# CompVis/unsupervised-part-segmentation

Measured on AMD Instinct MI355X. Metric: images/sec training (CUB 128x128, 10 parts), higher is better.
Workload: dtype bf16

## Files before the change

unsupervised-part-segmentation_amd/csrc/conv_igemm.hip:

```cpp
#include <stdlib.h>

#include "common.h"

namespace {

constexpr int BM = 128;
constexpr int RS = 80;

template <typename T> struct Mma;

template <> struct Mma<bf16> {
    template <int TM, int TN>
    __device__ static inline void chunk(const unsigned char* a_base, const unsigned char* b_base, int lane,
                                        f32x16 (&acc)[TM][TN]) {
        const int r = lane & 31, h = lane >> 5;
#pragma unroll
        for (int ks = 0; ks < 2; ++ks) {
            bf16x8 a[TM], b[TN];
#pragma unroll
            for (int i = 0; i < TM; ++i) a[i] = *(const bf16x8*)(a_base + (i * 32 + r) * RS + ks * 32 + h * 16);
#pragma unroll
            for (int j = 0; j < TN; ++j) b[j] = *(const bf16x8*)(b_base + (j * 32 + r) * RS + ks * 32 + h * 16);
#pragma unroll
            for (int i = 0; i < TM; ++i)
#pragma unroll
                for (int j = 0; j < TN; ++j)
                    acc[i][j] = __builtin_amdgcn_mfma_f32_32x32x16_bf16(a[i], b[j], acc[i][j], 0, 0, 0);
        }
    }
};

template <> struct Mma<f16> {
    template <int TM, int TN>
    __device__ static inline void chunk(const unsigned char* a_base, const unsigned char* b_base, int lane,
                                        f32x16 (&acc)[TM][TN]) {
        const int r = lane & 31, h = lane >> 5;
#pragma unroll
        for (int ks = 0; ks < 2; ++ks) {
            f16x8 a[TM], b[TN];
#pragma unroll
            for (int i = 0; i < TM; ++i) a[i] = *(const f16x8*)(a_base + (i * 32 + r) * RS + ks * 32 + h * 16);
#pragma unroll
            for (int j = 0; j < TN; ++j) b[j] = *(const f16x8*)(b_base + (j * 32 + r) * RS + ks * 32 + h * 16);
#pragma unroll
            for (int i = 0; i < TM; ++i)
#pragma unroll
                for (int j = 0; j < TN; ++j)
                    acc[i][j] = __builtin_amdgcn_mfma_f32_32x32x16_f16(a[i], b[j], acc[i][j], 0, 0, 0);
        }
    }
};

template <> struct Mma<float> {
    template <int TM, int TN>
    __device__ static inline void chunk(const unsigned char* a_base, const unsigned char* b_base, int lane,
                                        f32x16 (&acc)[TM][TN]) {
        const int r = lane & 31, h = lane >> 5;
        f32x4 a[TM][2], b[TN][2];
#pragma unroll
        for (int i = 0; i < TM; ++i) {
            a[i][0] = *(const f32x4*)(a_base + (i * 32 + r) * RS + h * 32);
            a[i][1] = *(const f32x4*)(a_base + (i * 32 + r) * RS + h * 32 + 16);
        }
#pragma unroll
        for (int j = 0; j < TN; ++j) {
            b[j][0] = *(const f32x4*)(b_base + (j * 32 + r) * RS + h * 32);
            b[j][1] = *(const f32x4*)(b_base + (j * 32 + r) * RS + h * 32 + 16);
        }
#pragma unroll
        for (int kk = 0; kk < 8; ++kk)
#pragma unroll
            for (int i = 0; i < TM; ++i)
#pragma unroll
                for (int j = 0; j < TN; ++j)
                    acc[i][j] = __builtin_amdgcn_mfma_f32_32x32x2f32(a[i][kk >> 2][kk & 3], b[j][kk >> 2][kk & 3],
                                                                     acc[i][j], 0, 0, 0);
    }
};

__device__ inline int tap_dy_of(unsigned long long off, int t) { return (int)((off >> (4 * t + 2)) & 3) - 1; }
__device__ inline int tap_dx_of(unsigned long long off, int t) { return (int)((off >> (4 * t)) & 3) - 1; }
__device__ inline int tap_w_of(unsigned long long wi, int t) { return (int)((wi >> (4 * t)) & 15); }

struct ConvK {
    int n, hi, wi, ci, ldi, ho, wo, co, co_fill, ldo, out_h, out_w, out_sy, out_sx, out_oy, out_ox, in_sy, in_sx;
    int ntaps, kh, kw, act_in, out_f32, dact_kind, ldr, ldd, out_act, res_act;
    float act_slope;
    unsigned long long tap_off, tap_wi;
    const void* in; const void* w; void* out;
    const float* bias; const float* coord_tab; const void* res; const void* dact;
    float* ws; int splits, stages_per_split, ldw;
};

template <typename T, int BN, int CPS>
__global__ __launch_bounds__(256, (CPS == 1 ? 3 : 2)) void conv_igemm_kernel(const ConvK p, const int M, const int ntn,
                                                         const int kchunks) {
    constexpr int EPC = Chunk<T>::N;
    constexpr int BK = 4 * EPC;
    constexpr int WN = (BN == 32) ? 1 : 2;
    constexpr int WM = 4 / WN;
    constexpr int TM = BM / WM / 32;
    constexpr int TN = BN / WN / 32;
    constexpr int BROWS = (BN + 63) / 64;

    constexpr int SUB = (BM + BN) * RS;
    constexpr int STAGE = CPS * SUB;
    extern __shared__ __attribute__((aligned(16))) unsigned char smem[];
    long long* rowpix = (long long*)(smem + 2 * STAGE);
    int* rowaux = (int*)(rowpix + BM);

    const int tid = threadIdx.x, lane = tid & 63, wid = tid >> 6;
    const float act_ns = ups_slope_eff(p.act_in, p.act_slope);
    const float dact_ns = ups_slope_eff(p.dact_kind, p.act_slope);
    const int nt = blockIdx.x % ntn, mt = blockIdx.x / ntn;
    const int wm = wid / WN, wn = wid % WN;

    const T* __restrict__ in = (const T*)p.in;
    const T* __restrict__ w = (const T*)p.w;
    const int hw_o = p.ho * p.wo;

    const int chunk = tid & 3, r0 = tid >> 2;
    int iy0[2], ix0[2];
    long long ibase[2];
    bool rv[2];
#pragma unroll
    for (int q = 0; q < 2; ++q) {
        const int m = mt * BM + r0 + 64 * q;
        rv[q] = m < M;
        const int mm = rv[q] ? m : 0;
        const int img = mm / hw_o, rem = mm - img * hw_o;
        const int i = rem / p.wo, j = rem - i * p.wo;
        iy0[q] = i * p.in_sy;
        ix0[q] = j * p.in_sx;
        ibase[q] = (long long)img * p.hi * p.wi;
    }
    const bool b_thread = (BN >= 64) || (tid < 128);

    struct RSet { uint4 a0[CPS], a1[CPS], b0[CPS], b1[CPS]; } s0, s1;
    const uint4 zero4 = make_uint4(0u, 0u, 0u, 0u);
    const int iy00 = iy0[0], iy01 = iy0[1], ix00 = ix0[0], ix01 = ix0[1];
    const long long ib0 = ibase[0], ib1 = ibase[1];
    const bool rv0 = rv[0], rv1 = rv[1];
    const int total = p.ntaps * kchunks;

    auto load_a = [&](bool rvq, int iy, int ix, long long ib, int dy, int dx, int koff, bool kok) __attribute__((always_inline)) -> uint4 {
        const int y = iy + dy, x = ix + dx;
        const bool ok = rvq && kok && (unsigned)y < (unsigned)p.hi && (unsigned)x < (unsigned)p.wi;
        uint4 v = zero4;
        if (ok) v = *(const uint4*)(in + ((ib + (long long)y * p.wi + x) * p.ldi + koff));
        return v;
    };
    auto load_b = [&](const T* wt, int c, bool live) __attribute__((always_inline)) -> uint4 {
        uint4 v = zero4;
        if (live && b_thread && c < p.co) v = *(const uint4*)(wt + (long long)c * BK + chunk * EPC);
        return v;
    };
    auto load_stage = [&](RSet& q, int sidx) __attribute__((always_inline)) {
#pragma unroll
        for (int u = 0; u < CPS; ++u) {
            const int c = sidx * CPS + u;
            const bool live = c < total;
            const int cs = live ? c : 0;
            const int t = cs / kchunks, kc = cs - t * kchunks;
            const int koff = kc * BK + chunk * EPC;
            const bool kok = live && koff < p.ci;
            const int dy = tap_dy_of(p.tap_off, t), dx = tap_dx_of(p.tap_off, t);
            q.a0[u] = load_a(rv0, iy00, ix00, ib0, dy, dx, koff, kok);
            q.a1[u] = load_a(rv1, iy01, ix01, ib1, dy, dx, koff, kok);
            const T* wt = w + ((long long)tap_w_of(p.tap_wi, t) * kchunks + kc) * p.co * BK;
            q.b0[u] = load_b(wt, nt * BN + r0, live);
            if (BROWS > 1) q.b1[u] = load_b(wt, nt * BN + r0 + 64, live);
        }
    };
    auto act_u4 = [&](uint4 u) __attribute__((always_inline)) -> uint4 {
        if (p.act_in != UPS_ACT_NONE) {
            u = ups_act_chunk(u, act_ns, (T*)nullptr);
        }
        return u;
    };
    auto store_stage = [&](const RSet& q, unsigned char* st) __attribute__((always_inline)) {
#pragma unroll
        for (int u = 0; u < CPS; ++u) {
            unsigned char* As = st + u * SUB;
            unsigned char* Bs = As + BM * RS;
            *(uint4*)(As + r0 * RS + chunk * 16) = act_u4(q.a0[u]);
            *(uint4*)(As + (r0 + 64) * RS + chunk * 16) = act_u4(q.a1[u]);
            if (b_thread) {
                *(uint4*)(Bs + r0 * RS + chunk * 16) = q.b0[u];
                if (BROWS > 1) *(uint4*)(Bs + (r0 + 64) * RS + chunk * 16) = q.b1[u];
            }
        }
    };

    f32x16 acc[TM][TN];
#pragma unroll
    for (int i = 0; i < TM; ++i)
#pragma unroll
        for (int j = 0; j < TN; ++j)
#pragma unroll
            for (int e = 0; e < 16; ++e) acc[i][j][e] = 0.f;

    const int all_stages = (total + CPS - 1) / CPS;
    const int sbase = p.splits > 1 ? blockIdx.y * p.stages_per_split : 0;
    const int nstages = p.splits > 1 ? min(p.stages_per_split, all_stages - sbase) : all_stages;
    load_stage(s0, sbase);
    store_stage(s0, smem);
    if (nstages > 1) load_stage(s1, sbase + 1);
    __syncthreads();
    auto iter = [&](int sidx, RSet& ld_set, const RSet& st_set) __attribute__((always_inline)) {
        if (sidx + 2 < nstages) load_stage(ld_set, sbase + sidx + 2);
        const unsigned char* st = smem + (sidx & 1) * STAGE;
#pragma unroll
        for (int u = 0; u < CPS; ++u)
            Mma<T>::template chunk<TM, TN>(st + u * SUB + (wm * TM * 32) * RS, st + u * SUB + BM * RS + (wn * TN * 32) * RS,
                                           lane, acc);
        if (sidx + 1 < nstages) store_stage(st_set, smem + ((sidx + 1) & 1) * STAGE);
        __syncthreads();
    };
    for (int sidx = 0; sidx < nstages; sidx += 2) {
        iter(sidx, s0, s1);
        if (sidx + 1 < nstages) iter(sidx + 1, s1, s0);
    }

    if (p.splits > 1) {
        float* wsp = p.ws + ((long long)blockIdx.y * M) * p.ldw;
#pragma unroll
        for (int tn = 0; tn < TN; ++tn) {
            const int col = nt * BN + (wn * TN + tn) * 32 + (lane & 31);
#pragma unroll
            for (int tm = 0; tm < TM; ++tm)
#pragma unroll
                for (int e = 0; e < 16; ++e) {
                    const int m = mt * BM + (wm * TM + tm) * 32 + (e & 3) + 8 * (e >> 2) + 4 * (lane >> 5);
                    if (m < M) wsp[(long long)m * p.ldw + col] = acc[tm][tn][e];
                }
        }
        return;
    }
    if (tid < BM) {
        const int m = mt * BM + tid;
        long long pix = -1;
        int cls = 0, i = 0, j = 0;
        if (m < M) {
            const int img = m / hw_o, rem = m - img * hw_o;
            i = rem / p.wo; j = rem - i * p.wo;
            pix = ((long long)img * p.out_h + (i * p.out_sy + p.out_oy)) * p.out_w + (j * p.out_sx + p.out_ox);
            if (p.coord_tab) {
                int ym = 0, xm = 0;
                for (int r = 0; r < p.kh; ++r) ym |= ((unsigned)(i * p.in_sy + tap_dy_of(p.tap_off, r * p.kw)) < (unsigned)p.hi) << r;
                for (int s = 0; s < p.kw; ++s) xm |= ((unsigned)(j * p.in_sx + tap_dx_of(p.tap_off, s)) < (unsigned)p.wi) << s;
                cls = ym * 8 + xm;
            }
        }
        rowpix[tid] = pix;
        rowaux[tid * 3 + 0] = cls; rowaux[tid * 3 + 1] = j; rowaux[tid * 3 + 2] = i;
    }
    __syncthreads();

    T* __restrict__ outT = (T*)p.out;
    float* __restrict__ outF = (float*)p.out;
    const T* __restrict__ res = (const T*)p.res;
    const T* __restrict__ dact = (const T*)p.dact;
#pragma unroll
    for (int tn = 0; tn < TN; ++tn) {
        const int col = nt * BN + (wn * TN + tn) * 32 + (lane & 31);
        const bool cvalid = col < p.co;
        const bool cfill = col < p.co_fill;
        const float bias = (cvalid && p.bias) ? p.bias[col] : 0.f;
#pragma unroll
        for (int tm = 0; tm < TM; ++tm) {
#pragma unroll
            for (int e = 0; e < 16; ++e) {
                const int rl = (wm * TM + tm) * 32 + (e & 3) + 8 * (e >> 2) + 4 * (lane >> 5);
                const long long pix = rowpix[rl];
                if (pix < 0 || !cfill) continue;
                float v = 0.f;
                if (cvalid) {
                    v = acc[tm][tn][e] + bias;
                    if (p.coord_tab) {
                        const float* tb = p.coord_tab + (long long)rowaux[rl * 3] * 3 * p.co + col;
                        v += tb[0] + (float)rowaux[rl * 3 + 1] * tb[p.co] + (float)rowaux[rl * 3 + 2] * tb[2 * p.co];
                    }
                    if (dact) v *= (ld_as_float<T>(dact + pix * p.ldd + col) > 0.f) ? 1.f : dact_ns;
                    if (res) {
                        float rr = ld_as_float<T>(res + pix * p.ldr + col);
                        if (p.res_act) rr = rr > 0.f ? rr : rr / p.act_slope;
                        v += rr;
                    }
                    if (p.out_act) v = ups_vmax(v, ups_slope_eff(p.out_act, p.act_slope) * v);
                }
                if (p.out_f32) outF[pix * p.ldo + col] = v;
                else st_from_float<T>(outT + pix * p.ldo + col, v);
            }
        }
    }
}

template <typename T>
__global__ __launch_bounds__(256) void igemm_splitk_epilogue(const ConvK p, const int M) {
    const long long gid = (long long)blockIdx.x * blockDim.x + threadIdx.x;
    const int col = (int)(gid % p.co_fill);
    const long long m = gid / p.co_fill;
    if (m >= M) return;
    float v = 0.f;
    for (int sp = 0; sp < p.splits; ++sp) v += p.ws[((long long)sp * M + m) * p.ldw + col];
    const int hw_o = p.ho * p.wo;
    const int img = (int)(m / hw_o), rem = (int)(m - (long long)img * hw_o);
    const int i = rem / p.wo, j = rem - i * p.wo;
    const long long pix = ((long long)img * p.out_h + (i * p.out_sy + p.out_oy)) * p.out_w + (j * p.out_sx + p.out_ox);
    const bool cvalid = col < p.co;
    if (cvalid) {
        if (p.bias) v += p.bias[col];
        if (p.coord_tab) {
            int ym = 0, xm = 0;
            for (int r = 0; r < p.kh; ++r) ym |= ((unsigned)(i * p.in_sy + tap_dy_of(p.tap_off, r * p.kw)) < (unsigned)p.hi) << r;
            for (int q = 0; q < p.kw; ++q) xm |= ((unsigned)(j * p.in_sx + tap_dx_of(p.tap_off, q)) < (unsigned)p.wi) << q;
            const float* tb = p.coord_tab + (long long)(ym * 8 + xm) * 3 * p.co + col;
            v += tb[0] + (float)j * tb[p.co] + (float)i * tb[2 * p.co];
        }
        if (p.dact) v *= (ld_as_float<T>((const T*)p.dact + pix * p.ldd + col) > 0.f) ? 1.f : ups_slope_eff(p.dact_kind, p.act_slope);
        if (p.res) {
            float rr = ld_as_float<T>((const T*)p.res + pix * p.ldr + col);
            if (p.res_act) rr = rr > 0.f ? rr : rr / p.act_slope;
            v += rr;
        }
        if (p.out_act) v = ups_vmax(v, ups_slope_eff(p.out_act, p.act_slope) * v);
    } else {
        v = 0.f;
    }
    if (p.out_f32) ((float*)p.out)[pix * p.ldo + col] = v;
    else st_from_float<T>((T*)p.out + pix * p.ldo + col, v);
}

template <typename T>
int launch(const ups_conv_desc& dd, hipStream_t s) {
    constexpr int EPC = Chunk<T>::N;
    ConvK d;
    d.n = dd.n; d.hi = dd.hi; d.wi = dd.wi; d.ci = dd.ci; d.ldi = dd.ldi; d.ho = dd.ho; d.wo = dd.wo; d.co = dd.co;
    d.co_fill = dd.co_fill; d.ldo = dd.ldo; d.out_h = dd.out_h; d.out_w = dd.out_w; d.out_sy = dd.out_sy;
    d.out_sx = dd.out_sx; d.out_oy = dd.out_oy; d.out_ox = dd.out_ox; d.in_sy = dd.in_sy; d.in_sx = dd.in_sx;
    d.ntaps = dd.ntaps; d.kh = dd.kh; d.kw = dd.kw; d.act_in = dd.act_in; d.out_f32 = dd.out_f32;
    d.dact_kind = dd.dact_kind; d.ldr = dd.ldr; d.ldd = dd.ldd; d.act_slope = dd.act_slope;
    d.out_act = dd.out_act; d.res_act = dd.res_act;
    d.in = dd.in; d.w = dd.w; d.out = dd.out; d.bias = dd.bias; d.coord_tab = dd.coord_tab; d.res = dd.res; d.dact = dd.dact;
    d.tap_off = 0; d.tap_wi = 0;
    for (int t = 0; t < dd.ntaps; ++t) {
        if (dd.tap_dy[t] < -1 || dd.tap_dy[t] > 2 || dd.tap_dx[t] < -1 || dd.tap_dx[t] > 2 || dd.tap_w[t] < 0 || dd.tap_w[t] > 15)
            return UPS_E_ARG;
        d.tap_off |= (unsigned long long)(((dd.tap_dy[t] + 1) << 2) | (dd.tap_dx[t] + 1)) << (4 * t);
        d.tap_wi |= (unsigned long long)dd.tap_w[t] << (4 * t);
    }
    const long long M = (long long)d.n * d.ho * d.wo;
    if (M <= 0 || M > 0x7fffffffLL) return UPS_E_ARG;
    const int kchunks = ups_cdiv(d.ci, 4 * EPC);
    const int ctot = d.co_fill;
    const int mtiles = ups_cdiv(M, BM);
    int bn = ctot > 64 ? 128 : (ctot > 32 ? 64 : 32);
    if (bn == 128 && mtiles * ups_cdiv(ctot, 128) < 256) bn = 64;
    if (bn == 64 && mtiles * ups_cdiv(ctot, 64) < 256) bn = 32;
    static int fbn = -1, fcps = 0;
    if (fbn < 0) {
        const char* e = getenv("UPS_IGEMM_FORCE");
        int a = 0, b = 0;
        if (e && sscanf(e, "%d,%d", &a, &b) == 2 && b > 0) fcps = b;
        fbn = a > 0 ? a : 0;
    }
    if (fbn > 0) bn = fbn;
    const int ntn = ups_cdiv(ctot, bn);
    const bool skinny = mtiles * ntn < 1024 && d.ntaps * kchunks >= 8;
    int cps = !skinny ? 1 : (bn == 32 ? 4 : (bn == 64 ? 2 : 1));
    if (fcps > 0) cps = fcps;
    d.ws = nullptr; d.splits = 1; d.stages_per_split = 0; d.ldw = 0;
    {
        static int sk_on = -1;
        if (sk_on < 0) { const char* e = getenv("UPS_NO_SPLITK"); sk_on = (e && e[0] == '1') ? 0 : 1; }
        const int chunks = d.ntaps * kchunks;
        const int bn_sk = ctot > 32 ? 64 : 32;
        const int blocks_sk = mtiles * ups_cdiv(ctot, bn_sk);
        const bool few = blocks_sk < 192 && chunks >= 16;
        const bool longk = (blocks_sk <= 320 && chunks >= 64) || (blocks_sk <= 512 && chunks >= 128);
        if (sk_on && dd.workspace && (few || longk)) {
            const int cps_sk = bn_sk == 64 ? 2 : 4;
            const int stages = ups_cdiv(chunks, cps_sk);
            int splits = ups_cdiv(few ? 512 : 1024, blocks_sk);
            if (splits > stages / 2) splits = stages / 2;
            const int sps = ups_cdiv(stages, splits);
            splits = ups_cdiv(stages, sps);
            const int ldw = ups_cdiv(ctot, bn_sk) * bn_sk;
            const size_t need = (size_t)splits * (size_t)M * ldw * sizeof(float);
            if (splits >= 2 && need <= dd.workspace_bytes) {
                bn = bn_sk; d.ws = dd.workspace; d.splits = splits; d.stages_per_split = sps; d.ldw = ldw;
            }
        }
    }
    const int ntn_l = ups_cdiv(ctot, bn);
    const int cps_l = d.splits > 1 ? (bn == 64 ? 2 : 4) : cps;
#define UPS_LAUNCH_IG(BNV, CPSV)                                                                                      \
    do {                                                                                                              \
        const size_t shmem = 2 * (size_t)(CPSV) * (BM + (BNV)) * RS + BM * 20;                                        \
        static UpsPerDevice attr_done;                                                                                \
        if (!attr_done) {                                                                                             \
            if (hipFuncSetAttribute((const void*)conv_igemm_kernel<T, BNV, CPSV>,                                     \
                                    hipFuncAttributeMaxDynamicSharedMemorySize, (int)shmem) != hipSuccess)           \
                return UPS_E_LAUNCH;                                                                                  \
            attr_done = true;                                                                                         \
        }                                                                                                             \
        hipLaunchKernelGGL((conv_igemm_kernel<T, BNV, CPSV>), dim3(mtiles * ntn_l, d.splits), dim3(256), shmem, s, d,  \
                           (int)M, ntn_l, kchunks);                                                                   \
    } while (0)
    if (bn == 128) UPS_LAUNCH_IG(128, 1);
    else if (bn == 64 && cps_l == 2) UPS_LAUNCH_IG(64, 2);
    else if (bn == 64) UPS_LAUNCH_IG(64, 1);
    else if (cps_l == 4) UPS_LAUNCH_IG(32, 4);
    else UPS_LAUNCH_IG(32, 1);
#undef UPS_LAUNCH_IG
    if (d.splits > 1) {
        const long long elems = M * (long long)d.co_fill;
        hipLaunchKernelGGL((igemm_splitk_epilogue<T>), dim3(ups_cdiv(elems, 256)), dim3(256), 0, s, d, (int)M);
    }
    return UPS_OK;
}

}

int ups_conv3x3_patch_try(const ups_conv_desc* d, hipStream_t s);
bool ups_conv3x3_patch_signs(const ups_conv_desc* d);
extern "C" int ups_sign_pack(const void* x, int32_t dtype, int64_t chunks, void* sign_bits, void* stream);

thread_local int g_ups_sign_written = 0;
extern "C" int ups_conv_sign_out_written(void) { return g_ups_sign_written; }
int ups_conv3x3_first_try(const ups_conv_desc* d, hipStream_t s);
int ups_conv3x3_s2_try(const ups_conv_desc* d, hipStream_t s);
int ups_conv3x3_rows_try(const ups_conv_desc* d, hipStream_t s);
int ups_conv3x3_rows_s2_try(const ups_conv_desc* d, hipStream_t s);
int ups_conv3x3_thinout_try(const ups_conv_desc* d, hipStream_t s);
int ups_conv3x3_rows_maskgrad_try(const ups_conv_desc* d, hipStream_t s);

extern "C" int ups_conv_igemm(const ups_conv_desc* d, void* stream) {
    UPS_CHECK_ARG(d != nullptr);
    g_ups_sign_written = 0;
    UPS_CHECK_ARG(d->dtype == UPS_F32 || d->dtype == UPS_BF16 || d->dtype == UPS_F16);
    UPS_CHECK_ARG(d->in && d->w && (d->out || d->mask_grad));
    if (d->dtype == UPS_F16 && (d->d2s || d->f8_deq || d->mask_bits || d->mask_grad || d->in_f8 || d->out_f8 || d->out_f8_amax)) {
        ups_set_error("ups_conv_igemm: UPS_F16 is a forward format: no fp8 copies, part masks or depth-to-space output");
        return UPS_E_UNSUPPORTED;
    }
    UPS_CHECK_ARG(d->ci > 0 && d->ci % 8 == 0 && d->ldi % 8 == 0 && d->ci <= d->ldi);
    UPS_CHECK_ARG(d->ntaps >= 1 && d->ntaps <= 9);
    UPS_CHECK_ARG(d->act_slope >= 0.f && d->act_slope <= 1.f);
    UPS_CHECK_ARG(d->out_act >= UPS_ACT_NONE && d->out_act <= UPS_ACT_RELU);
    UPS_CHECK_ARG(d->res_act == UPS_ACT_NONE || (d->res_act == UPS_ACT_LRELU && d->act_slope > 0.f && d->res));
    UPS_CHECK_ARG(d->co >= 1 && d->co_fill >= d->co && (d->d2s ? d->d2s <= d->ldo : d->co_fill <= d->ldo));
    UPS_CHECK_ARG(d->n > 0 && d->ho > 0 && d->wo > 0 && d->hi > 0 && d->wi > 0);
    UPS_CHECK_ARG(!d->coord_tab || (d->kh * d->kw == d->ntaps && d->kh <= 3 && d->kw <= 3));
    UPS_CHECK_ARG(((uintptr_t)d->in & 15) == 0 && ((uintptr_t)d->w & 15) == 0);
    UPS_CHECK_ARG((d->out_sy * (d->ho - 1) + d->out_oy) < d->out_h && (d->out_sx * (d->wo - 1) + d->out_ox) < d->out_w);
    if (d->sign_out) {
        UPS_CHECK_ARG(d->dtype != UPS_F32 && !d->out_f32 && (d->ldo & 7) == 0 && d->out && !d->d2s && !d->mask_grad);
        UPS_CHECK_ARG(d->out_sy == 1 && d->out_sx == 1 && !d->out_oy && !d->out_ox && d->out_h == d->ho && d->out_w == d->wo);
    }
    const char* force = getenv("UPS_FORCE_GENERIC_CONV");
    if (!(force && force[0] == '1')) {
        if (ups_conv3x3_first_try(d, (hipStream_t)stream) == 0) { UPS_LAUNCH_CHECK(); return UPS_OK; }
        {
            const int rr = ups_conv3x3_rows_s2_try(d, (hipStream_t)stream);
            if (rr == 0) { UPS_LAUNCH_CHECK(); return UPS_OK; }
            if (rr < 0) { ups_set_error("ups_conv_igemm: row-streaming stride-2 kernel launch setup failed"); return rr; }
        }
        {
            const int sr = ups_conv3x3_s2_try(d, (hipStream_t)stream);
            if (sr == 0) { UPS_LAUNCH_CHECK(); return UPS_OK; }
            if (sr < 0) { ups_set_error("ups_conv_igemm: stride-2 kernel launch setup failed"); return sr; }
        }
        {
            int rr = ups_conv3x3_thinout_try(d, (hipStream_t)stream);
            if (rr == 1) rr = ups_conv3x3_rows_try(d, (hipStream_t)stream);
            if (rr == 1) rr = ups_conv3x3_rows_maskgrad_try(d, (hipStream_t)stream);
            if (rr == 0) { UPS_LAUNCH_CHECK(); return UPS_OK; }
            if (rr < 0) { ups_set_error("ups_conv_igemm: row-streaming kernel launch setup failed"); return rr; }
        }
        const int pr = ups_conv3x3_patch_try(d, (hipStream_t)stream);
        if (pr == 0) { UPS_LAUNCH_CHECK(); if (d->sign_out && ups_conv3x3_patch_signs(d)) g_ups_sign_written = 1; return UPS_OK; }
        if (pr < 0) { ups_set_error("ups_conv_igemm: patch kernel launch setup failed"); return pr; }
    }
    if (d->d2s) {
        ups_set_error("ups_conv_igemm: the depth-to-space output needs the bf16 3x3 / stride-1 patch kernel (16-aligned lattice, 4 x 2^k channels)");
        return UPS_E_UNSUPPORTED;
    }
    if (d->f8_deq) {
        ups_set_error("ups_conv_igemm: the fp8 forward needs the bf16 3x3 / stride-1 patch kernel (16-aligned images, ci %% 64 == 0, no mask)");
        return UPS_E_UNSUPPORTED;
    }
    if (d->mask_bits || d->mask_grad) {
        ups_set_error("ups_conv_igemm: the part-masked forms need the bf16 3x3 / stride-1 patch kernel (16-aligned images, P <= 32)");
        return UPS_E_UNSUPPORTED;
    }
    if (d->out_f8 || d->out_f8_amax || d->in_f8) {
        ups_set_error("ups_conv_igemm: fp8 copies (in_f8 / out_f8 / out_f8_amax) need the bf16 3x3 / stride-1 patch kernel");
        return UPS_E_UNSUPPORTED;
    }
    int rc = (d->dtype == UPS_F32) ? launch<float>(*d, (hipStream_t)stream)
             : (d->dtype == UPS_F16 ? launch<f16>(*d, (hipStream_t)stream) : launch<bf16>(*d, (hipStream_t)stream));
    if (rc != UPS_OK) { ups_set_error("ups_conv_igemm: bad problem size"); return rc; }
    UPS_LAUNCH_CHECK();
    return UPS_OK;
}
```

unsupervised-part-segmentation_amd/switches.py:

```python
import os
from collections import OrderedDict

SWITCHES = OrderedDict([
    ("UPS_LIB", ("", "ab", "lib.py", "path of the library to load instead of csrc/libupsparts_hip.so (A/B builds: tools/ab_build.sh)")),
    ("UPS_DIST_BACKEND", ("nccl", "product", "runner.py", "torch.distributed backend (nccl = RCCL; gloo for the CPU / one-GPU tests)")),
    ("UPS_GRAPH", ("0", "product", "model.py", "1: HIP-graph replay of the step (config key hip_graph)")),
    ("UPS_STREAM_PLAN", ("auto", "product", "model.py", "full | compact | auto: side-stream budget (config key stream_plan; DESIGN section 7)")),
    ("UPS_NO_OVERLAP", ("0", "ab", "ops.py", "1: everything on one stream (per-kernel profiles without CU sharing)")),
    ("UPS_POST_ACT", ("1", "ab", "nets.py", "0: activation-on-load everywhere instead of post-activation storage (config key post_activation_storage)")),
    ("UPS_SIGN_BITS", ("1", "ab", "ops.py", "0: input gradients read the forward input for act' instead of the producer's sign bytes")),
    ("UPS_VGG_FP8", ("0", "ab", "model.py", "1: fp8 copies through the perceptual trunk (config key vgg_fp8; measured slower, DESIGN 3b)")),
    ("UPS_F8_WGRAD", ("1", "ab", "ops.py", "0: bf16 weight gradients in precision fp8")),
    ("UPS_F8_PRODUCER", ("1", "ab", "ops.py", "0: fp8 copies converted by a separate pass instead of the producing epilogue")),
    ("UPS_TOWERS", ("1", "ab", "ops.py", "0: the critics' towers through the generic convolution path instead of the grouped launches")),
    ("UPS_STATE_KERNEL", ("1", "ab", "model.py", "0: the Lagrangian / EMA state update as ~30 torch launches instead of one kernel")),
    ("UPS_LATE_JOIN", ("1", "ab", "model.py", "0: a single rank joins the weight-gradient stream at every segment boundary")),
    ("UPS_EARLY_ADAM", ("1", "ab", "model.py", "0: every key's Adam at the end of the step instead of behind its weight gradients")),
    ("UPS_EARLY_ALPHA", ("1", "ab", "model.py", "0: the appearance code after the pose encoder instead of beside it on `aux`")),
    ("UPS_CRITIC_STREAMS", ("1", "ab", "model.py", "0: the three critics on one stream")),
    ("UPS_COORD_STREAM", ("1", "ab", "ops.py", "0: the CoordConv rows of the weight gradients on the weight-gradient stream itself")),
    ("UPS_NO_D2S", ("0", "ab", "ops.py", "1: the stride-2 layers' input gradient as four phase launches instead of one depth-to-space launch")),
    ("UPS_DP_SIDE_LAUNCH", ("1", "ab", "model.py", "0: bucket all-reduces launched from the launching stream (it then waits for the weight gradients)")),
    ("UPS_DP_STANDIN", ("0", "debug", "dist.py", "1: every bucket all-reduce replaced by a device copy on its own stream (one-GPU stream-budget probe)")),
    ("UPS_FORCE_COLLECTIVES", ("0", "test", "dist.py", "1: issue the collectives at world size 1 (the RCCL call pattern test)")),
    ("UPS_JOIN_TIMING", ("0", "debug", "model.py", "1: HIP events around the end-of-backward joins (tools/probes/join_wait.py)")),
    ("UPS_ROWS_KERNEL", ("1", "test", "conv3x3_rows.hip", "0: row-stream layers through the patch / generic kernels; force: also at small batches (parity tests)")),
    ("UPS_S2_KERNEL", ("1", "ab", "conv3x3_s2.hip", "0: the other stride-2 forwards through the generic kernel")),
    ("UPS_THIN_SW", ("32", "ab", "conv3x3_rows.hip", "16: 16-column strips in the logit convolution (measured equal)")),
    ("UPS_FIRST_LAYER", ("1", "ab", "conv3x3_first.hip", "0: the 3-channel first layers through the generic kernel")),
    ("UPS_FORCE_GENERIC_CONV", ("0", "test", "conv_igemm.hip", "1: every convolution through the generic gather kernel")),
    ("UPS_IGEMM_FORCE", ("", "test", "conv_igemm.hip", "tile variant of the generic kernel")),
    ("UPS_NO_SPLITK", ("0", "ab", "conv_igemm.hip", "1: no split-K for the small-grid generic launches")),
    ("UPS_NO_SMALL_PATCH", ("0", "ab", "conv3x3_patch.hip", "1: no small-tile patch instances")),
    ("UPS_PATCH_CST", ("", "ab", "conv3x3_patch.hip", "patch kernel: constant-stride instances on / off")),
    ("UPS_PATCH_DMA", ("1", "ab", "conv3x3_patch.hip", "0: register-staged patches instead of LDS-DMA")),
    ("UPS_PATCH_MID", ("", "ab", "conv3x3_patch.hip", "patch kernel: mid-size tile selection")),
    ("UPS_PATCH_OCC", ("", "ab", "conv3x3_patch.hip", "patch kernel: blocks per CU override")),
    ("UPS_PATCH_RAGGED", ("1", "ab", "conv3x3_patch.hip", "0: images that are not a multiple of 16 leave the patch kernel")),
    ("UPS_PATCH_STATIC", ("", "ab", "conv3x3_patch.hip", "patch kernel: static-geometry instances on / off")),
    ("UPS_PATCH_THIN128", ("", "ab", "conv3x3_patch.hip", "patch kernel: thin 128-wide instance selection")),
    ("UPS_PATCH_THINOUT", ("", "ab", "conv3x3_patch.hip", "patch kernel: thin-output instance selection")),
    ("UPS_RES_PATCH", ("1", "ab", "conv3x3_patch.hip", "0: the forward's residual from global memory instead of the resident patch")),
    ("UPS_RES_PATCH_DGRAD", ("1", "ab", "conv3x3_patch.hip", "0: the input gradient's residual and sign bytes fetched in the epilogue instead of from the resident patch (round 6)")),
    ("UPS_F8_SCALED", ("1", "ab", "conv3x3_patch.hip", "0: K = 32 fp8 MFMA instead of the block-scaled K = 128 form")),
    ("UPS_WGRAD_DIRECT", ("1", "ab", "conv_wgrad.hip", "0: single-split weight gradients through a slab + reduce launch")),
    ("UPS_WGRAD_SLIDE", ("1", "ab", "conv_wgrad3x3.hip", "0: the plain form of the 3x3 weight gradient (3 % slower step)")),
    ("UPS_PRIOR_PX", ("1", "ab", "priors.hip", "0: the staged prior kernels at P = 10 instead of the pixel-per-lane rings")),
    ("UPS_PRIOR_PX_BPI", ("", "test", "priors.hip", "cap on blocks per image of the pixel-per-lane prior kernels (multi-tile loops at three images)")),
    ("UPS_PRIOR_DIRECT", ("1", "ab", "priors.hip", "0: the staged prior kernels at P = 16 / 20 / 25 instead of the chunk-per-lane direct-from-global forms (round 6)")),
    ("UPS_SOFTMAX_PX", ("1", "ab", "partpath.hip", "0: the LDS-walking soft-max kernel at P = 10")),
    ("UPS_MOMENTS_PX", ("1", "ab", "partpath.hip", "0: the slab form of the spatial moments at P = 10")),
    ("UPS_MOMENTS_PX_BLOCKS", ("", "test", "partpath.hip", "blocks of the pixel-per-lane moments kernel")),
    ("UPS_UNPOOL_MFMA", ("1", "test", "partpath.hip", "0: the VALU form of unpool_bwd (the unit test compares both)")),
])

COMPILE_TIME = ("UPS_ROWS_FWD_SIGN", "UPS_ROWS_NO_FENCE", "UPS_VMAX_BUILTIN")
NOT_SWITCHES = ("UPS_ABI_VERSION", "UPS_ACT_", "UPS_OK", "UPS_E_", "UPS_BF16", "UPS_F16", "UPS_F32", "UPS_CHECK_ARG", "UPS_LAUNCH_CHECK")


def value(name):
    return os.environ.get(name, SWITCHES[name][0])


def flag(name):
    d = SWITCHES[name][0]
    v = os.environ.get(name, d)
    return v != "0" if d == "1" else v == "1"


def report():
    diff = ["{}={}".format(k, os.environ[k]) for k, (d, _, _, _) in SWITCHES.items() if k in os.environ and os.environ[k] != d]
    return "UPS switches: " + (", ".join(diff) if diff else "all defaults")
```

Before: 2121.

## Add thin-input 3x3 conv kernel with register-resident weights for wide outputs

Adds a specialised bf16 3x3 stride-1 kernel for layers with 8/16/32 input channels and up to 512 output channels, such as the logit convolution's input gradient. Each wave keeps all tap weights in registers, packs several taps into one K=32 MFMA, and streams 16-pixel groups with a one-ahead prefetch, writing outputs directly (optional LDS-transposed epilogue). It applies the activation derivative from sign bits in the epilogue. The goal is to replace the patch kernel, which wastes work on a single thin input chunk, with a persistent output-write-bound stream. The cost is extra code paths and possibly uncoalesced direct stores.

```diff
diff --git a/unsupervised-part-segmentation_amd/csrc/conv3x3_thinin.hip b/unsupervised-part-segmentation_amd/csrc/conv3x3_thinin.hip
--- /dev/null
+++ b/unsupervised-part-segmentation_amd/csrc/conv3x3_thinin.hip
@@ -0,0 +1,197 @@
+#include "common.h"
+#include <stdlib.h>
+
+namespace {
+
+struct ThinK {
+    const bf16* in; const bf16* w; bf16* out;
+    const unsigned char* bits;
+    int h, wd, ldi, co, ldo, ldb;
+    int gpr;
+    long long groups;
+    int ncg, streams;
+    int all_valid;
+    float ns;
+    unsigned long long tap_off, tap_wi;
+};
+
+template <int CI> struct ThinCfg {
+    static constexpr int MT = CI == 32 ? 2 : 4;
+    static constexpr int TPS = 32 / CI;
+    static constexpr int NS = (9 + TPS - 1) / TPS;
+    static constexpr int OCC = CI == 8 ? 4 : 3;
+};
+
+template <int CI, bool DACT, bool LDS_EPI>
+__global__ void __launch_bounds__(256, ThinCfg<CI>::OCC) conv3x3_thinin_kernel(const ThinK p) {
+    constexpr int MT = ThinCfg<CI>::MT, TPS = ThinCfg<CI>::TPS, NS = ThinCfg<CI>::NS;
+    constexpr int ERS = MT * 32 + 16;
+    __shared__ __attribute__((aligned(16))) unsigned char stage[LDS_EPI ? 4 * 16 * ERS : 16];
+    const int lane = threadIdx.x & 63, pl = lane & 15, q = lane >> 4;
+    const int wave = __builtin_amdgcn_readfirstlane((int)(threadIdx.x >> 6));
+    const int total = gridDim.x, hb = blockIdx.x;
+    const int lb = (hb & 7) * (total >> 3) + (hb >> 3);
+    const int gw = lb * 4 + wave;
+    const int st = gw / p.ncg, cg = gw - st * p.ncg;
+    const int chbase = cg * (16 * MT);
+    if (st >= p.streams) return;
+
+    int boff[NS], bdy[NS], bdx[NS];
+    bf16x8 A[NS][MT];
+    const bf16x8 zero8 = __builtin_bit_cast(bf16x8, make_uint4(0u, 0u, 0u, 0u));
+#pragma unroll
+    for (int s = 0; s < NS; ++s) {
+        const int ts = (8 * q) / CI, ch = (8 * q) % CI, t = s * TPS + ts;
+        const bool tv = t < 9;
+        const int tt = tv ? t : 0;
+        const int code = (int)((p.tap_off >> (4 * tt)) & 15ull), tw = (int)((p.tap_wi >> (4 * tt)) & 15ull);
+        const int dy = (code >> 2) - 1, dx = (code & 3) - 1;
+        bdy[s] = tv ? dy : (1 << 24);
+        bdx[s] = dx;
+        boff[s] = (dy * p.wd + dx) * p.ldi + ch;
+#pragma unroll
+        for (int m = 0; m < MT; ++m) {
+            const int c = chbase + 32 * (m >> 1) + 8 * (pl >> 2) + 4 * (m & 1) + (pl & 3);
+            A[s][m] = (tv && c < p.co) ? *(const bf16x8*)(p.w + ((long long)(tw * p.co + c) * 32 + ch)) : zero8;
+        }
+    }
+
+    const long long g0 = p.groups * st / p.streams, g1 = p.groups * (st + 1) / p.streams;
+    if (g0 >= g1) return;
+    long long row = g0 / p.gpr;
+    int xg = (int)(g0 - row * p.gpr), y = (int)(row % p.h);
+
+    bf16x8 Bn[NS];
+    unsigned sgn[2] = {0u, 0u};
+    unsigned okn = 0u;
+    long long pixn = 0;
+    auto fetch = [&]() __attribute__((always_inline)) {
+        pixn = row * p.wd + xg * 16;
+        const bf16* src = p.in + pixn * p.ldi + pl * p.ldi;
+        okn = 0u;
+#pragma unroll
+        for (int s = 0; s < NS; ++s) {
+            const bool ok = (unsigned)(y + bdy[s]) < (unsigned)p.h && (unsigned)(xg * 16 + pl + bdx[s]) < (unsigned)p.wd;
+            Bn[s] = *(const bf16x8*)(src + (ok ? boff[s] : 0));
+            okn |= ok ? 1u << s : 0u;
+        }
+        if constexpr (DACT) {
+            const unsigned char* sp = p.bits + (pixn + pl) * p.ldb + (chbase >> 3);
+            if constexpr (MT == 4) { const uint2 v = *(const uint2*)sp; sgn[0] = v.x; sgn[1] = v.y; }
+            else sgn[0] = *(const unsigned*)sp;
+        }
+    };
+    fetch();
+    for (long long g = g0; g < g1; ++g) {
+        bf16x8 B[NS];
+#pragma unroll
+        for (int s = 0; s < NS; ++s) B[s] = (okn >> s) & 1u ? Bn[s] : zero8;
+        const unsigned sg0 = sgn[0], sg1 = sgn[1];
+        const long long pix = pixn;
+        if (g + 1 < g1) {
+            if (++xg == p.gpr) { xg = 0; ++row; if (++y == p.h) y = 0; }
+        }
+        fetch();
+
+        f32x4 acc[MT];
+#pragma unroll
+        for (int m = 0; m < MT; ++m) acc[m] = (f32x4){0.f, 0.f, 0.f, 0.f};
+#pragma unroll
+        for (int s = 0; s < NS; ++s)
+#pragma unroll
+            for (int m = 0; m < MT; ++m) acc[m] = __builtin_amdgcn_mfma_f32_16x16x32_bf16(A[s][m], B[s], acc[m], 0, 0, 0);
+
+        bf16* orow = p.out + (pix + pl) * p.ldo + chbase + 8 * q;
+#pragma unroll
+        for (int u = 0; u < MT / 2; ++u) {
+            float v[8];
+#pragma unroll
+            for (int e = 0; e < 4; ++e) { v[e] = acc[2 * u][e]; v[4 + e] = acc[2 * u + 1][e]; }
+            if constexpr (DACT) {
+                const unsigned db = ((u ? sg1 : sg0) >> (8 * q)) & 0xffu;
+#pragma unroll
+                for (int e = 0; e < 8; ++e) v[e] *= (db >> e) & 1u ? 1.f : p.ns;
+            }
+            if (!p.all_valid) {
+                const int c = chbase + 32 * u + 8 * q;
+#pragma unroll
+                for (int e = 0; e < 8; ++e) if (c + e >= p.co) v[e] = 0.f;
+            }
+            const uint4 o = Chunk<bf16>::pack(v);
+            if constexpr (LDS_EPI) *(uint4*)(stage + wave * (16 * ERS) + pl * ERS + 64 * u + 16 * q) = o;
+            else *(uint4*)(orow + 32 * u) = o;
+        }
+        if constexpr (LDS_EPI) {
+            constexpr int LPP = MT * 2, PPI = 64 / LPP;
+            const int px = lane / LPP, chk = lane - px * LPP;
+#pragma unroll
+            for (int i = 0; i < 16 / PPI; ++i) {
+                const uint4 o = *(const uint4*)(stage + wave * (16 * ERS) + (i * PPI + px) * ERS + 16 * chk);
+                *(uint4*)(p.out + (pix + i * PPI + px) * p.ldo + chbase + 8 * chk) = o;
+            }
+        }
+    }
+}
+
+template <int CI>
+int thinin_launch(ThinK& k, int co_fill, int cus, bool dact, bool lds_epi, hipStream_t s) {
+    constexpr int MT = ThinCfg<CI>::MT;
+    k.ncg = co_fill / (16 * MT);
+    const int unit = 8 * k.ncg;
+    int blocks = (cus * ThinCfg<CI>::OCC / unit) * unit;
+    if (blocks < unit) blocks = unit;
+    k.streams = blocks * 4 / k.ncg;
+    if ((long long)k.streams > k.groups) return 1;
+#define UPS_THININ_LAUNCH(D, E) hipLaunchKernelGGL((conv3x3_thinin_kernel<CI, D, E>), dim3((unsigned)blocks), dim3(256), 0, s, k)
+    if (dact) { if (lds_epi) UPS_THININ_LAUNCH(true, true); else UPS_THININ_LAUNCH(true, false); }
+    else { if (lds_epi) UPS_THININ_LAUNCH(false, true); else UPS_THININ_LAUNCH(false, false); }
+#undef UPS_THININ_LAUNCH
+    return 0;
+}
+
+}
+
+int ups_conv3x3_thinin_try(const ups_conv_desc* d, hipStream_t s) {
+    { const char* e = getenv("UPS_THININ"); if (e && e[0] == '0') return 1; }
+    if (d->dtype != UPS_BF16 || d->ntaps != 9 || d->in_sy != 1 || d->in_sx != 1 || d->out_sy != 1 || d->out_sx != 1 || d->out_oy ||
+        d->out_ox || d->hi != d->ho || d->wi != d->wo || d->out_h != d->ho || d->out_w != d->wo)
+        return 1;
+    if (!(d->ci == 8 || d->ci == 16 || d->ci == 32) || d->co_fill % 128 || d->co_fill > 512 || d->co > d->co_fill || (d->ldo & 7) ||
+        (d->hi % 16) || (d->wi % 16))
+        return 1;
+    if (d->out_f32 || d->d2s || d->mask_bits || d->mask_grad || d->coord_tab || d->bias || d->res || d->res_act || d->out_act ||
+        d->act_in != UPS_ACT_NONE || d->f8_deq || d->in_f8 || d->out_f8 || d->out_f8_amax || d->sign_out || !d->out)
+        return 1;
+    if (d->dact && (!d->dact_bits || (d->ldd & 63) || d->ldd < d->co_fill || (((uintptr_t)d->dact_bits) & 7))) return 1;
+    if (((uintptr_t)d->out) & 15) return 1;
+    const long long tiles = (long long)d->n * (d->hi / 16) * (d->wi / 16);
+    if (tiles * (d->co_fill / 128) < 512) return 1;
+    if (((long long)d->wi + 2) * d->ldi * 2 >= (1ll << 30) || (long long)d->n * d->hi * d->wi >= (1ll << 40)) return 1;
+    bool seen[9] = {false, false, false, false, false, false, false, false, false};
+    ThinK k;
+    k.tap_off = 0; k.tap_wi = 0;
+    for (int t = 0; t < 9; ++t) {
+        const int dy = d->tap_dy[t], dx = d->tap_dx[t];
+        if (dy < -1 || dy > 1 || dx < -1 || dx > 1 || d->tap_w[t] < 0 || d->tap_w[t] > 15) return 1;
+        seen[(dy + 1) * 3 + dx + 1] = true;
+        k.tap_off |= (unsigned long long)(((dy + 1) << 2) | (dx + 1)) << (4 * t);
+        k.tap_wi |= (unsigned long long)d->tap_w[t] << (4 * t);
+    }
+    for (int t = 0; t < 9; ++t) if (!seen[t]) return 1;
+    k.in = (const bf16*)d->in; k.w = (const bf16*)d->w; k.out = (bf16*)d->out;
+    k.bits = d->dact ? (const unsigned char*)d->dact_bits : nullptr;
+    k.h = d->hi; k.wd = d->wi; k.ldi = d->ldi; k.co = d->co; k.ldo = d->ldo; k.ldb = d->ldd >> 3;
+    k.gpr = d->wi / 16;
+    k.groups = (long long)d->n * d->hi * k.gpr;
+    k.all_valid = d->co == d->co_fill;
+    k.ns = d->dact_kind == UPS_ACT_LRELU ? d->act_slope : 0.f;
+    int dev = 0, cus = 0;
+    if (hipGetDevice(&dev) != hipSuccess || hipDeviceGetAttribute(&cus, hipDeviceAttributeMultiprocessorCount, dev) != hipSuccess || cus <= 0)
+        return UPS_E_LAUNCH;
+    bool lds_epi = false;
+    { const char* e = getenv("UPS_THININ_EPI"); lds_epi = e && e[0] == 'l'; }
+    const bool dact = d->dact != nullptr;
+    if (d->ci == 8) return thinin_launch<8>(k, d->co_fill, cus, dact, lds_epi, s);
+    if (d->ci == 16) return thinin_launch<16>(k, d->co_fill, cus, dact, lds_epi, s);
+    return thinin_launch<32>(k, d->co_fill, cus, dact, lds_epi, s);
+}
diff --git a/unsupervised-part-segmentation_amd/csrc/conv_igemm.hip b/unsupervised-part-segmentation_amd/csrc/conv_igemm.hip
--- a/unsupervised-part-segmentation_amd/csrc/conv_igemm.hip
+++ b/unsupervised-part-segmentation_amd/csrc/conv_igemm.hip
@@ -435,6 +435,7 @@
 int ups_conv3x3_rows_s2_try(const ups_conv_desc* d, hipStream_t s);
 int ups_conv3x3_thinout_try(const ups_conv_desc* d, hipStream_t s);
 int ups_conv3x3_rows_maskgrad_try(const ups_conv_desc* d, hipStream_t s);
+int ups_conv3x3_thinin_try(const ups_conv_desc* d, hipStream_t s);
 
 extern "C" int ups_conv_igemm(const ups_conv_desc* d, void* stream) {
     UPS_CHECK_ARG(d != nullptr);
@@ -479,6 +480,11 @@
             if (rr == 0) { UPS_LAUNCH_CHECK(); return UPS_OK; }
             if (rr < 0) { ups_set_error("ups_conv_igemm: row-streaming kernel launch setup failed"); return rr; }
         }
+        {
+            const int tr = ups_conv3x3_thinin_try(d, (hipStream_t)stream);
+            if (tr == 0) { UPS_LAUNCH_CHECK(); return UPS_OK; }
+            if (tr < 0) { ups_set_error("ups_conv_igemm: thin-in kernel launch setup failed"); return tr; }
+        }
         const int pr = ups_conv3x3_patch_try(d, (hipStream_t)stream);
         if (pr == 0) { UPS_LAUNCH_CHECK(); if (d->sign_out && ups_conv3x3_patch_signs(d)) g_ups_sign_written = 1; return UPS_OK; }
         if (pr < 0) { ups_set_error("ups_conv_igemm: patch kernel launch setup failed"); return pr; }
diff --git a/unsupervised-part-segmentation_amd/switches.py b/unsupervised-part-segmentation_amd/switches.py
--- a/unsupervised-part-segmentation_amd/switches.py
+++ b/unsupervised-part-segmentation_amd/switches.py
@@ -27,6 +27,8 @@
     ("UPS_ROWS_KERNEL", ("1", "test", "conv3x3_rows.hip", "0: row-stream layers through the patch / generic kernels; force: also at small batches (parity tests)")),
     ("UPS_S2_KERNEL", ("1", "ab", "conv3x3_s2.hip", "0: the other stride-2 forwards through the generic kernel")),
     ("UPS_THIN_SW", ("32", "ab", "conv3x3_rows.hip", "16: 16-column strips in the logit convolution (measured equal)")),
+    ("UPS_THININ", ("1", "ab", "conv3x3_thinin.hip", "0: single-chunk wide-output 3x3 layers (the logit convolution's input gradient) through the patch kernel instead of the output-write stream")),
+    ("UPS_THININ_EPI", ("", "ab", "conv3x3_thinin.hip", "lds: the thin-in kernel stores through a wave-private LDS transposition instead of straight from the accumulators (docs/design/kernels.md)")),
     ("UPS_FIRST_LAYER", ("1", "ab", "conv3x3_first.hip", "0: the 3-channel first layers through the generic kernel")),
     ("UPS_FORCE_GENERIC_CONV", ("0", "test", "conv_igemm.hip", "1: every convolution through the generic gather kernel")),
     ("UPS_IGEMM_FORCE", ("", "test", "conv_igemm.hip", "tile variant of the generic kernel")),
```

After: 2132, median of 6. About the same (+0.5%).
